# Artemarius/cuda-gaussian-splatting

Hardware: AMD Instinct MI355X
Metric: fwd+bwd Mpixels/s @1080p, 1M Gaussians, SH3 (higher is better)
Workload: dtype f32

## Files before the change

cuda-gaussian-splatting_amd/csrc/sort_bin.h:

```cpp
#pragma once

#include "sort_bin_cover.h"
#include "sort_tile_order.h"

namespace {

constexpr int BIN_WAVES = 16, BIN_NT = BIN_WAVES * CUGS_WAVE;
inline uint32_t bin_window_groups(int ntx) { const uint32_t nbx = ((uint32_t)ntx + 7u) / 8u; return (nbx + 7u) / 8u; }
inline uint32_t bin_window_cols(int ntx) {
    const uint32_t nbx = ((uint32_t)ntx + 7u) / 8u, gxs = bin_window_groups(ntx);
    return ((nbx + gxs - 1u) / gxs) * 8u;
}
inline uint32_t bin_windows(int ntx, int nty) { return (((uint32_t)nty + 7u) / 8u) * bin_window_groups(ntx); }

constexpr int BIN_D_MAX = BIN_TILES_CAP + 2 * CUGS_PRECT_MAX_TILES + 2;
__global__ __launch_bounds__(BIN_NT) void k_bin_count(uint32_t n, uint32_t group, const uint32_t* __restrict__ order,
                                                      const int4* __restrict__ rect, const uint32_t* __restrict__ prect_in,
                                                      uint32_t* __restrict__ prect_out, uint32_t ntx, uint32_t nty,
                                                      uint32_t* __restrict__ table, uint32_t* __restrict__ zero_pairs,
                                                      uint32_t* __restrict__ win) {
    __shared__ int32_t s_d[BIN_D_MAX];
    if (blockIdx.x == 0 && threadIdx.x < BIN_WINDOWS_MAX) win[threadIdx.x] = 0u;
    __shared__ int32_t s_part[8][128];
    const uint32_t tid = threadIdx.x, wave = tid >> 6, lane = tid & 63u;
    const uint32_t w2 = ntx + 1u, cells = w2 * (nty + 1u);
    for (uint32_t e = tid; e < cells; e += BIN_NT) s_d[e] = 0;
    __syncthreads();
    const uint32_t base = blockIdx.x * group;
    const uint32_t end = min(n, base + group);
    for (uint32_t i = base + tid; i < end; i += BIN_NT) {
        uint32_t pr;
        if (prect_in) {
            pr = prect_in[i];
        } else {
            pr = pack_rect(rect[order[i]]);
            prect_out[i] = pr;
        }
        if (pr & 0x80000000u) {
            const uint32_t z = pr & 0x7FFFFFFFu;
            if (z) atomicAdd(zero_pairs, z);
            continue;
        }
        const uint32_t x0 = pr & 127u, y0 = (pr >> 7) & 127u, w = (pr >> 14) & 127u, h = (pr >> 21) & 127u;
        atomicAdd(&s_d[y0 * w2 + x0], 1);
        atomicAdd(&s_d[y0 * w2 + x0 + w], -1);
        atomicAdd(&s_d[(y0 + h) * w2 + x0], -1);
        atomicAdd(&s_d[(y0 + h) * w2 + x0 + w], 1);
    }
    __syncthreads();
    for (uint32_t row = wave; row < nty; row += BIN_WAVES) {
        int32_t carry = 0;
        for (uint32_t c0 = 0; c0 < ntx; c0 += CUGS_WAVE) {
            const uint32_t x = c0 + lane;
            const int32_t v = x < ntx ? s_d[row * w2 + x] : 0;
            const int32_t inc = (int32_t)wave_inclusive_scan((uint32_t)v) + carry;
            if (x < ntx) s_d[row * w2 + x] = inc;
            carry = __shfl(inc, 63);
        }
    }
    __syncthreads();
    {
        const uint32_t x = tid & 127u, seg = tid >> 7;
        const uint32_t rps = (nty + 7u) / 8u;
        const uint32_t ya = min(nty, seg * rps), yb = min(nty, ya + rps);
        int32_t sum = 0;
        if (x < ntx)
            for (uint32_t y = ya; y < yb; ++y) sum += s_d[y * w2 + x];
        s_part[seg][x] = sum;
        __syncthreads();
        int32_t run = 0;
        for (uint32_t s2 = 0; s2 < seg; ++s2) run += s_part[s2][x];
        if (x < ntx)
            for (uint32_t y = ya; y < yb; ++y) {
                run += s_d[y * w2 + x];
                s_d[y * w2 + x] = run;
            }
    }
    __syncthreads();
    uint32_t* out = table + (size_t)blockIdx.x * (ntx * nty);
    for (uint32_t row = wave; row < nty; row += BIN_WAVES)
        for (uint32_t x = lane; x < ntx; x += CUGS_WAVE) out[row * ntx + x] = (uint32_t)s_d[row * w2 + x];
}

__global__ __launch_bounds__(BIN_NT) void k_bin_scan(uint32_t rows, uint32_t tiles, uint32_t* __restrict__ table,
                                                     uint32_t* __restrict__ ttot, uint32_t* __restrict__ tpre,
                                                     uint32_t* __restrict__ csum, uint32_t* __restrict__ q12,
                                                     uint32_t* __restrict__ range_flag, uint32_t* __restrict__ snap,
                                                     uint32_t* __restrict__ win, uint32_t ntx, uint32_t win_cols,
                                                     uint32_t gxs) {
    __shared__ uint32_t s_seg[BIN_WAVES][CUGS_WAVE];
    __shared__ uint32_t s_win[BIN_WINDOWS_MAX];
    if (blockIdx.x == 0 && threadIdx.x == 0) {
        snap[0] = q12[0]; q12[1] = q12[0]; q12[0] = 0u;
        snap[1] = *range_flag; *range_flag = 0u;
    }
    const uint32_t tl = threadIdx.x & 63u, seg = threadIdx.x >> 6;
    const uint32_t t = blockIdx.x * CUGS_WAVE + tl;
    const uint32_t rps = (rows + BIN_WAVES - 1u) / BIN_WAVES;
    const uint32_t r0 = min(rows, seg * rps), r1 = min(rows, r0 + rps);
    uint32_t sum = 0u;
    if (t < tiles) {
#pragma unroll 8
        for (uint32_t r = r0; r < r1; ++r) sum += table[(size_t)r * tiles + t];
    }
    s_seg[seg][tl] = sum;
    __syncthreads();
    uint32_t pre = 0u, tot = 0u;
#pragma unroll
    for (uint32_t s2 = 0; s2 < (uint32_t)BIN_WAVES; ++s2) {
        const uint32_t v = s_seg[s2][tl];
        pre += s2 < seg ? v : 0u;
        tot += v;
    }
    if (t < tiles) {
        uint32_t run = pre;
#pragma unroll 8
        for (uint32_t r = r0; r < r1; ++r) {
            const uint32_t v = table[(size_t)r * tiles + t];
            table[(size_t)r * tiles + t] = run;
            run += v;
        }
    }
    if (seg == 0u) {
        const uint32_t v = t < tiles ? tot : 0u;
        const uint32_t inc = wave_inclusive_scan(v);
        if (t < tiles) { ttot[t] = v; tpre[t] = inc - v; }
        if (tl == 63u) csum[blockIdx.x] = inc;
        if (win) {
            s_win[tl] = 0u;
            __builtin_amdgcn_fence(__ATOMIC_ACQ_REL, "wavefront");
            __builtin_amdgcn_wave_barrier();
            if (v) {
                const uint32_t ty = t / ntx, tx = t - ty * ntx;
                atomicAdd(&s_win[(ty >> 3) * gxs + tx / win_cols], v);
            }
            __builtin_amdgcn_fence(__ATOMIC_ACQ_REL, "wavefront");
            __builtin_amdgcn_wave_barrier();
            const uint32_t mine = s_win[tl];
            if (mine) atomicAdd(&win[tl], mine);
        }
    }
}

constexpr int BIN_BLK = 8;
constexpr int BIN_WG_WAVES = 8;
constexpr int BIN_SLICE = 512;
constexpr int BIN_SLICE_STEPS = BIN_SLICE / CUGS_WAVE;
constexpr int BIN_RUN = 16;
constexpr int BIN_RUN_STRIDE = BIN_RUN + 3;
__device__ __forceinline__ void bin_wave_lds_sync() {
    __builtin_amdgcn_fence(__ATOMIC_ACQ_REL, "wavefront");
    __builtin_amdgcn_wave_barrier();
}
template <int CTRL>
__device__ __forceinline__ uint32_t bin_dpp(uint32_t v) {
    return (uint32_t)__builtin_amdgcn_update_dpp(0, (int)v, CTRL, 0xF, 0xF, false);
}
template <int S, uint32_t M>
__device__ __forceinline__ uint32_t bin_tr_merge(uint32_t v, uint32_t p, bool upper) {
    const uint32_t keep = upper ? ~M : M;
    const uint32_t moved = __builtin_rotateright32(p, upper ? (uint32_t)S : 32u - (uint32_t)S);
    return (v & keep) | (moved & ~keep);
}
__device__ __forceinline__ void bin_transpose64(uint32_t& lo, uint32_t& hi, uint32_t lane) {
    {
        const auto r = __builtin_amdgcn_permlane32_swap(lo, hi, false, false);
        lo = r[0]; hi = r[1];
    }
    {
        const bool up = (lane & 16u) != 0u;
        const uint32_t pl = (uint32_t)__shfl_xor((int)lo, 16), ph = (uint32_t)__shfl_xor((int)hi, 16);
        lo = bin_tr_merge<16, 0x0000FFFFu>(lo, pl, up); hi = bin_tr_merge<16, 0x0000FFFFu>(hi, ph, up);
    }
    {
        const bool up = (lane & 8u) != 0u;
        const uint32_t pl = bin_dpp<0x128>(lo), ph = bin_dpp<0x128>(hi);
        lo = bin_tr_merge<8, 0x00FF00FFu>(lo, pl, up); hi = bin_tr_merge<8, 0x00FF00FFu>(hi, ph, up);
    }
    {
        const bool up = (lane & 4u) != 0u;
        const uint32_t pl = bin_dpp<0x1B>(bin_dpp<0x141>(lo)), ph = bin_dpp<0x1B>(bin_dpp<0x141>(hi));
        lo = bin_tr_merge<4, 0x0F0F0F0Fu>(lo, pl, up); hi = bin_tr_merge<4, 0x0F0F0F0Fu>(hi, ph, up);
    }
    {
        const bool up = (lane & 2u) != 0u;
        const uint32_t pl = bin_dpp<0x4E>(lo), ph = bin_dpp<0x4E>(hi);
        lo = bin_tr_merge<2, 0x33333333u>(lo, pl, up); hi = bin_tr_merge<2, 0x33333333u>(hi, ph, up);
    }
    {
        const bool up = (lane & 1u) != 0u;
        const uint32_t pl = bin_dpp<0xB1>(lo), ph = bin_dpp<0xB1>(hi);
        lo = bin_tr_merge<1, 0x55555555u>(lo, pl, up); hi = bin_tr_merge<1, 0x55555555u>(hi, ph, up);
    }
}
__device__ __forceinline__ void bin_pop_batch(const uint2* hits, uint32_t count, uint32_t lane, uint32_t blk_tx0,
                                              uint32_t blk_ty0, bool tile_ok, char* outb, uint32_t& pos) {
    bin_wave_lds_sync();
    const uint64_t cover = lane < count ? bin_cover_mask(hits[lane].x, blk_tx0, blk_ty0) : 0ull;
    uint32_t lo = (uint32_t)cover, hi = (uint32_t)(cover >> 32);
    bin_transpose64(lo, hi, lane);
    if (!tile_ok) lo = hi = 0u;
    const uint32_t* const word = reinterpret_cast<const uint32_t*>(hits);
    while (lo != 0u) {
        const uint32_t b = (uint32_t)__builtin_ctz(lo);
        lo &= lo - 1u;
        *reinterpret_cast<uint32_t*>(outb + pos) = word[2u * b + 1u];
        pos += 4u;
    }
    while (hi != 0u) {
        const uint32_t b = (uint32_t)__builtin_ctz(hi);
        hi &= hi - 1u;
        *reinterpret_cast<uint32_t*>(outb + pos) = word[2u * b + 65u];
        pos += 4u;
    }
    bin_wave_lds_sync();
}

template <bool STAGE>
__global__ __launch_bounds__(BIN_WG_WAVES * CUGS_WAVE) void k_bin_scatter(
    uint32_t n, uint32_t group, uint32_t nbx, uint32_t nby, uint32_t gxs, uint32_t pairs_or_cap, bool predicted,
    const uint32_t* __restrict__ order, const uint32_t* __restrict__ prect, uint32_t ntx, uint32_t nty,
    const uint32_t* __restrict__ table, const uint32_t* __restrict__ ttot, const uint32_t* __restrict__ tpre,
    const uint32_t* __restrict__ csum, const uint32_t* __restrict__ snap, uint32_t* __restrict__ tbase,
    unsigned long long* __restrict__ total, unsigned long long* __restrict__ total_mapped, uint32_t* __restrict__ out,
    int32_t* __restrict__ tile_ranges, uint32_t* __restrict__ tile_order, const uint32_t* __restrict__ win) {
    __shared__ uint2 s_cand[BIN_WG_WAVES][BIN_SLICE];
    __shared__ uint32_t s_cnt[BIN_WG_WAVES];
    __shared__ uint2 s_hit[STAGE ? 1 : BIN_WG_WAVES * CUGS_WAVE];
    __shared__ uint32_t s_run[STAGE ? BIN_WG_WAVES * CUGS_WAVE * BIN_RUN_STRIDE + 4 : 1];
    const uint32_t nt = blockDim.x, nw = nt >> 6, tid = threadIdx.x, wid = tid >> 6, lane = tid & 63u;
    const uint32_t per_group = nby * gxs;
    uint32_t blk = blockIdx.x / per_group, rem = blockIdx.x - blk * per_group;
    const uint32_t win_mine = (win && lane < per_group) ? win[lane] : 0u;
    const uint32_t zero = snap[0];
    const bool bad = snap[1] != 0u;
    const uint32_t tiles = ntx * nty;

    const uint32_t nch = (tiles + CUGS_WAVE - 1u) / CUGS_WAVE;
    uint32_t cpre[3] = {0u, 0u, 0u};
    uint32_t pairs = zero;
#pragma unroll
    for (int i = 0; i < 3; ++i) {
        if ((uint32_t)i * CUGS_WAVE < nch) {
            const uint32_t c = lane + (uint32_t)i * CUGS_WAVE;
            const uint32_t v = c < nch ? csum[c] : 0u;
            uint32_t inc = v;
#pragma unroll
            for (int d = 1; d < 64; d <<= 1) {
                const uint32_t o = __shfl_up(inc, d);
                const uint32_t sum = inc + o;
                if ((int)lane >= d) inc = sum < o ? 0xFFFFFFFFu : sum;
            }
            const uint32_t with = inc + pairs;
            cpre[i] = (with < inc ? 0xFFFFFFFFu : with) - v;
            const uint32_t last = __shfl(inc, 63), tot = last + pairs;
            pairs = tot < last ? 0xFFFFFFFFu : tot;
        }
    }
    const bool fits = !bad && (!predicted || pairs <= pairs_or_cap);
    cpre[0] -= zero; cpre[1] -= zero; cpre[2] -= zero;
    if (__ballot((unsigned long long)win_mine * per_group > 2ull * pairs) != 0ull) {
        uint32_t rank = 0u;
        for (uint32_t w2 = 0; w2 < per_group; ++w2) {
            const uint32_t o = (uint32_t)__builtin_amdgcn_readlane((int)win_mine, (int)w2);
            rank += (o > win_mine || (o == win_mine && w2 < lane)) ? 1u : 0u;
        }
        const uint32_t groups = gridDim.x / per_group;
        const uint32_t slot = blockIdx.x / groups;
        blk = blockIdx.x - slot * groups;
        rem = (uint32_t)__builtin_ctzll(__ballot(lane < per_group && rank == slot));
    }
    const uint32_t by = rem / gxs, gx = rem - by * gxs;

    const uint32_t bx = gx * nw + wid;
    const bool active = bx < nbx;
    const uint32_t tx = bx * BIN_BLK + (lane & 7u), ty = by * BIN_BLK + (lane >> 3);
    const bool tile_ok = active && tx < ntx && ty < nty;
    const uint32_t t = tile_ok ? ty * ntx + tx : 0u;
    uint32_t start;
    {
        const uint32_t ch = t >> 6;
        const uint32_t p0 = __shfl(cpre[0], ch & 63u), p1 = __shfl(cpre[1], ch & 63u), p2 = __shfl(cpre[2], ch & 63u);
        start = zero + (ch < 64u ? p0 : ch < 128u ? p1 : p2) + (tile_ok ? tpre[t] : 0u);
    }
    uint32_t pos = tile_ok ? (start + table[(size_t)blk * tiles + t]) * 4u : 0u;
    if (blk == 0u) {
        if (tile_ok) {
            const uint32_t c = fits ? ttot[t] + (t == 0u ? zero : 0u) : 0u;
            tile_ranges[2 * t + 0] = c ? (int32_t)(t == 0u ? 0u : start) : 0;
            tile_ranges[2 * t + 1] = c ? (int32_t)(start + ttot[t]) : 0;
            tbase[t] = start;
        }
        if (rem == 0u && tid == 0u) {
            unsigned long long exact = zero;
            for (uint32_t c = 0; c < nch; ++c) exact += csum[c];
            tbase[tiles] = pairs;
            const unsigned long long host_total = bad ? ~0ull : exact;
            total[0] = bad ? 0ull : exact;
            total[1] = host_total;
            if (total_mapped) __hip_atomic_store(total_mapped, host_total, __ATOMIC_RELAXED, __HIP_MEMORY_SCOPE_SYSTEM);
        }
    }
    if (tile_order && blockIdx.x == 0u) {
        uint32_t* const s_lds = reinterpret_cast<uint32_t*>(&s_cand[0][0]);
        uint32_t* const s_chunk = s_lds + ORDER_LDS;
        if (wid == 0u) {
#pragma unroll
            for (int i = 0; i < 3; ++i)
                if (lane + (uint32_t)i * CUGS_WAVE < nch) s_chunk[lane + (uint32_t)i * CUGS_WAVE] = cpre[i];
        }
        write_tile_order(tiles, [&](uint32_t t2) { return fits ? ttot[t2] + (t2 == 0u ? zero : 0u) : 0u; },
                         [&](uint32_t t2) { return t2 == 0u ? 0u : zero + s_chunk[t2 >> 6] + tpre[t2]; },
                         reinterpret_cast<uint4*>(tile_order), s_lds);
    }
    if (!fits) return;
    if (blk == 0u)
        for (uint32_t k = rem * nt + tid; k < zero; k += per_group * nt) out[k] = 0u;
    const uint32_t win_y0 = by * BIN_BLK, win_y1 = win_y0 + BIN_BLK;
    const uint32_t win_x0 = gx * nw * BIN_BLK, win_x1 = win_x0 + nw * BIN_BLK;
    const uint32_t blk_x0 = bx * BIN_BLK, blk_x1 = blk_x0 + BIN_BLK;
    const unsigned long long lt_mask = (1ull << lane) - 1ull;
    char* const outb = reinterpret_cast<char*>(out);
    uint32_t* const run = s_run + (STAGE ? tid * BIN_RUN_STRIDE : 0u);
    uint32_t held = 0u;
    uint2* const hits = s_hit + (STAGE ? 0u : wid * CUGS_WAVE);
    uint32_t nhit = 0u;
    const uint32_t base = blk * group;
    const uint32_t end = min(n, base + group);
    const uint32_t stage = nw * BIN_SLICE;
    for (uint32_t c0 = base; c0 < end; c0 += stage) {
        __syncthreads();
        {
            const uint32_t s_begin = c0 + wid * BIN_SLICE;
            uint32_t pr[BIN_SLICE_STEPS], gq[BIN_SLICE_STEPS];
            bool ov[BIN_SLICE_STEPS];
#pragma unroll
            for (int u = 0; u < BIN_SLICE_STEPS; ++u) {
                const uint32_t i = s_begin + (uint32_t)u * CUGS_WAVE + lane;
                pr[u] = prect[min(i, end - 1u)];
                gq[u] = order[min(i, end - 1u)];
                if (i >= end) pr[u] = 0x80000000u;
            }
#pragma unroll
            for (int u = 0; u < BIN_SLICE_STEPS; ++u) {
                const uint32_t x0 = pr[u] & 127u, y0 = (pr[u] >> 7) & 127u, w = (pr[u] >> 14) & 127u, h = (pr[u] >> 21) & 127u;
                ov[u] = (int32_t)pr[u] >= 0 && y0 < win_y1 && y0 + h > win_y0 && x0 < win_x1 && x0 + w > win_x0;
            }
            uint32_t found = 0u;
#pragma unroll
            for (int u = 0; u < BIN_SLICE_STEPS; ++u) {
                const unsigned long long m = __ballot(ov[u]);
                if (ov[u]) s_cand[wid][found + (uint32_t)__popcll(m & lt_mask)] = make_uint2(pr[u], gq[u]);
                found += (uint32_t)__popcll(m);
            }
            if (lane == 0u) s_cnt[wid] = found;
        }
        __syncthreads();
        if (!active) continue;
        if constexpr (!STAGE) {
            const uint32_t cnts = s_cnt[lane & (uint32_t)(BIN_WG_WAVES - 1)];
            for (uint32_t w2 = 0; w2 < nw; ++w2) {
                const uint32_t c = (uint32_t)__builtin_amdgcn_readlane((int)cnts, (int)w2);
                for (uint32_t k0 = 0; k0 < c; k0 += CUGS_WAVE) {
                    const uint2 rec = s_cand[w2][k0 + lane];
                    const uint32_t x0v = rec.x & 127u, wv = (rec.x >> 14) & 127u;
                    const bool hit = k0 + lane < c && (int32_t)rec.x >= 0 && x0v < blk_x1 && x0v + wv > blk_x0;
                    const unsigned long long m = __builtin_amdgcn_ballot_w64(hit);
                    const uint32_t slot = __builtin_amdgcn_mbcnt_hi((uint32_t)(m >> 32), __builtin_amdgcn_mbcnt_lo((uint32_t)m, nhit));
                    if (hit && slot < (uint32_t)CUGS_WAVE) hits[slot] = rec;
                    nhit = (uint32_t)__builtin_amdgcn_readfirstlane((int)(nhit + (uint32_t)__popcll(m)));
                    if (nhit >= (uint32_t)CUGS_WAVE) {
                        bin_pop_batch(hits, (uint32_t)CUGS_WAVE, lane, blk_x0, win_y0, tile_ok, outb, pos);
                        if (hit && slot >= (uint32_t)CUGS_WAVE) hits[slot - (uint32_t)CUGS_WAVE] = rec;
                        nhit -= (uint32_t)CUGS_WAVE;
                    }
                }
            }
            continue;
        }
        for (uint32_t w2 = 0; w2 < nw; ++w2) {
            const uint32_t c = s_cnt[w2];
            for (uint32_t k0 = 0; k0 < c; k0 += CUGS_WAVE) {
                uint2 rec = make_uint2(0x80000000u, 0u);
                if (k0 + lane < c) rec = s_cand[w2][k0 + lane];
                const uint32_t x0v = rec.x & 127u, wv = (rec.x >> 14) & 127u;
                unsigned long long m = __ballot((int32_t)rec.x >= 0 && x0v < blk_x1 && x0v + wv > blk_x0);
                while (m != 0ull) {
                    const int l = __builtin_ctzll(m);
                    m &= m - 1ull;
                    const uint32_t prl = (uint32_t)__builtin_amdgcn_readlane((int)rec.x, l);
                    const uint32_t g = (uint32_t)__builtin_amdgcn_readlane((int)rec.y, l);
                    const uint32_t x0 = prl & 127u, y0 = (prl >> 7) & 127u, w = (prl >> 14) & 127u, h = (prl >> 21) & 127u;
                    const bool in = ((tx - x0) < w) & ((ty - y0) < h);
                    if constexpr (STAGE) {
                        if (in) run[held++] = g;
                        if (__ballot(held == (uint32_t)BIN_RUN) != 0ull) {
                            const uint32_t whole = held & ~3u;
#pragma unroll
                            for (int q = 0; q < BIN_RUN; q += 4)
                                if ((uint32_t)q < whole)
                                    *reinterpret_cast<uint4*>(outb + pos + 4 * q) = make_uint4(run[q], run[q + 1], run[q + 2], run[q + 3]);
                            const uint32_t rest = held - whole;
                            const uint32_t r0 = run[whole], r1 = run[whole + 1u], r2 = run[whole + 2u];
                            if (rest > 0u) run[0] = r0;
                            if (rest > 1u) run[1] = r1;
                            if (rest > 2u) run[2] = r2;
                            pos += 4u * whole;
                            held = rest;
                        }
                    } else if (in) {
                        *reinterpret_cast<uint32_t*>(outb + pos) = g;
                        pos += 4u;
                    }
                }
            }
        }
    }
    if constexpr (!STAGE) {
        if (nhit != 0u) bin_pop_batch(hits, nhit, lane, blk_x0, win_y0, tile_ok, outb, pos);
    }
    if constexpr (STAGE) {
        for (uint32_t q = 0; __ballot(q < held) != 0ull; ++q)
            if (q < held) *reinterpret_cast<uint32_t*>(outb + pos + 4u * q) = run[q];
    }
}

__global__ __launch_bounds__(CUGS_BLOCK) void k_bin_keys(uint32_t pairs_or_cap, const unsigned long long* __restrict__ dev_count,
                                                         uint32_t tiles, const uint32_t* __restrict__ tbase,
                                                         const uint32_t* __restrict__ zero_snap,
                                                         const int32_t* __restrict__ pidx, const float* __restrict__ depths,
                                                         uint64_t* __restrict__ keys_sorted) {
    if (dev_count && *dev_count > (unsigned long long)pairs_or_cap) return;
    const uint32_t total = live_count(pairs_or_cap, dev_count);
    const uint32_t i = blockIdx.x * CUGS_BLOCK + threadIdx.x;
    if (i >= total) return;
    if (i < *zero_snap) { keys_sorted[i] = 0ull; return; }
    uint32_t lo = 0u, hi = tiles;
    while (hi - lo > 1u) {
        const uint32_t mid = (lo + hi) >> 1;
        if (tbase[mid] <= i) lo = mid; else hi = mid;
    }
    keys_sorted[i] = ((uint64_t)lo << 32) | (uint64_t)__float_as_uint(depths[pidx[i]]);
}

}
```

cuda-gaussian-splatting_amd/csrc/sort_radix.h:

```cpp
#pragma once

#include "sort_workspace.h"

namespace {

__device__ __forceinline__ uint32_t wave_inclusive_scan(uint32_t v) {
    const int lane = threadIdx.x & 63;
#pragma unroll
    for (int d = 1; d < 64; d <<= 1) {
        uint32_t t = __shfl_up(v, d);
        if (lane >= d) v += t;
    }
    return v;
}

template <int NW = 4>
__device__ __forceinline__ uint32_t block_exclusive_scan(uint32_t v, uint32_t* s_tmp, uint32_t* total) {
    const int lane = threadIdx.x & 63, wave = threadIdx.x >> 6;
    uint32_t inc = wave_inclusive_scan(v);
    if (lane == 63) s_tmp[wave] = inc;
    __syncthreads();
    uint32_t base = 0, sum = 0;
#pragma unroll
    for (int w = 0; w < NW; ++w) {
        const uint32_t t = s_tmp[w];
        base += (w < wave) ? t : 0u;
        sum += t;
    }
    if (total) *total = sum;
    __syncthreads();
    return base + inc - v;
}

__device__ __forceinline__ uint32_t live_count(uint32_t count, const unsigned long long* __restrict__ dev_count) {
    if (!dev_count) return count;
    const unsigned long long t = *dev_count;
    return t < (unsigned long long)count ? (uint32_t)t : count;
}

template <typename K, int NT, int CHUNK, int RDX = RADIX>
__global__ __launch_bounds__(NT) void k_radix_hist(const K* __restrict__ keys, uint32_t count_or_cap,
                                                   const unsigned long long* __restrict__ dev_count, int shift,
                                                   uint32_t mask, uint32_t* __restrict__ hist, uint32_t nblk,
                                                   uint32_t* __restrict__ ctl, uint32_t* __restrict__ sup, uint32_t sb) {
    const uint32_t count = live_count(count_or_cap, dev_count);
    constexpr int PER = CHUNK / NT;
    constexpr int NWORDS = PER * (int)sizeof(K) / 4;
    static_assert(NWORDS >= 2 && NWORDS * 4 == PER * (int)sizeof(K), "whole 8-byte loads per thread");
    static_assert(NT >= RDX, "one thread per digit");
    __shared__ uint32_t s_cnt[RDX];
    if (threadIdx.x < RDX) s_cnt[threadIdx.x] = 0;
    if (ctl && blockIdx.x == 0 && threadIdx.x == 0) { ctl[1] = ctl[0]; ctl[0] = 0u; }
    __syncthreads();
    const uint32_t bbase = blockIdx.x * CHUNK;
    if (bbase + CHUNK <= count) {
        uint32_t wds[NWORDS];
        if constexpr (NWORDS % 4 == 0) {
            const uint4* src = reinterpret_cast<const uint4*>(keys + bbase + threadIdx.x * PER);
#pragma unroll
            for (int v = 0; v < NWORDS / 4; ++v) {
                const uint4 q = src[v];
                wds[4 * v] = q.x; wds[4 * v + 1] = q.y; wds[4 * v + 2] = q.z; wds[4 * v + 3] = q.w;
            }
        } else {
            const uint2* src = reinterpret_cast<const uint2*>(keys + bbase + threadIdx.x * PER);
#pragma unroll
            for (int v = 0; v < NWORDS / 2; ++v) {
                const uint2 q = src[v];
                wds[2 * v] = q.x; wds[2 * v + 1] = q.y;
            }
        }
#pragma unroll
        for (int c = 0; c < NWORDS; ++c) {
            if (sizeof(K) == 4) {
                atomicAdd(&s_cnt[(wds[c] >> shift) & mask], 1u);
            } else {
                atomicAdd(&s_cnt[((wds[c] & 0xFFFFu) >> shift) & mask], 1u);
                atomicAdd(&s_cnt[((wds[c] >> 16) >> shift) & mask], 1u);
            }
        }
    } else {
        for (uint32_t i = bbase + threadIdx.x; i < count; i += NT)
            atomicAdd(&s_cnt[((uint32_t)keys[i] >> shift) & mask], 1u);
    }
    __syncthreads();
    if (threadIdx.x < RDX) {
        const uint32_t c = s_cnt[threadIdx.x];
        if (sup) {
            hist[(size_t)blockIdx.x * RDX + threadIdx.x] = c;
            if (c) atomicAdd(&sup[(size_t)(blockIdx.x / sb) * RDX + threadIdx.x], c);
        } else {
            hist[(size_t)threadIdx.x * nblk + blockIdx.x] = c;
        }
    }
}

__global__ __launch_bounds__(CUGS_BLOCK) void k_radix_scan_rows(const uint32_t* hist, uint32_t* out,
                                                                uint32_t nblk, uint32_t* __restrict__ tot) {
    __shared__ uint32_t s_tmp[4];
    constexpr int PER = 8;
    const uint32_t* row = hist + (size_t)blockIdx.x * nblk;
    uint32_t* orow = out + (size_t)blockIdx.x * nblk;
    uint32_t carry = 0;
    for (uint32_t base = 0; base < nblk; base += CUGS_BLOCK * PER) {
        const uint32_t i0 = base + threadIdx.x * PER;
        uint32_t v[PER], sum = 0;
#pragma unroll
        for (int e = 0; e < PER; ++e) { v[e] = (i0 + e < nblk) ? row[i0 + e] : 0u; sum += v[e]; }
        uint32_t total;
        uint32_t run = carry + block_exclusive_scan(sum, s_tmp, &total);
#pragma unroll
        for (int e = 0; e < PER; ++e) {
            if (i0 + e < nblk) orow[i0 + e] = run;
            run += v[e];
        }
        carry += total;
    }
    if (threadIdx.x == 0) tot[blockIdx.x] = carry;
}

template <typename K, bool IOTA, int NB, int NT, bool ARANK, int CHUNK, int RDX = RADIX, bool V2 = false>
__global__ __launch_bounds__(NT) void k_radix_scatter(
    const K* __restrict__ keys_in, const uint32_t* __restrict__ vals_in, uint32_t count_or_cap,
    const unsigned long long* __restrict__ dev_count, int shift, uint32_t mask_rt, const uint32_t* __restrict__ hist,
    const uint32_t* __restrict__ sup, uint32_t sb, const uint32_t* __restrict__ tot, uint32_t nblk,
    K* __restrict__ keys_out, uint32_t* __restrict__ vals_out,
    const uint32_t* __restrict__ vals2_in = nullptr, uint32_t* __restrict__ vals2_out = nullptr) {
    const uint32_t mask = ARANK ? mask_rt : ((1u << NB) - 1u);
    const uint32_t count = live_count(count_or_cap, dev_count);
    if (blockIdx.x * CHUNK >= count) return;
    constexpr int NW = NT / CUGS_WAVE;
    constexpr int PER = CHUNK / NT;
    constexpr int SLICE = CUGS_WAVE * PER;
    static_assert(NT >= RDX && (1 << NB) <= RDX, "one thread per digit");
    __shared__ uint32_t s_lbase[NW][RDX];
    __shared__ uint32_t s_lstart[RDX];
    __shared__ uint32_t s_gbase[RDX];
    __shared__ K s_key[CHUNK];
    __shared__ uint32_t s_val[CHUNK];
    __shared__ uint32_t s_val2[V2 ? CHUNK : 1];
    __shared__ uint32_t s_tmp[NW];
    const uint32_t tid = threadIdx.x, wave = tid >> 6, lane = tid & 63;
    const uint32_t bbase = blockIdx.x * CHUNK;
    const uint32_t wbase = bbase + wave * SLICE;
    const uint32_t count_blk = min((uint32_t)CHUNK, count - bbase);

    constexpr int ND = ARANK ? RDX : (1 << NB);
    constexpr int GRP = NT / ND;
    uint32_t pre = 0u, totd = 0u;
    if (sup) {
        const uint32_t d = tid % ND, part = tid / ND;
        const uint32_t mysb = blockIdx.x / sb, nsb = (nblk + sb - 1u) / sb;
#pragma unroll 4
        for (uint32_t r = part; r < nsb; r += GRP) {
            const uint32_t v = sup[(size_t)r * RDX + d];
            totd += v;
            pre += (r < mysb) ? v : 0u;
        }
#pragma unroll 4
        for (uint32_t b2 = mysb * sb + part; b2 < blockIdx.x; b2 += GRP) pre += hist[(size_t)b2 * RDX + d];
    } else if (tid < RDX) {
        pre = hist[(size_t)tid * nblk + blockIdx.x];
        totd = tot[tid];
    }

    for (uint32_t e = tid; e < NW * RDX; e += NT) (&s_lbase[0][0])[e] = 0;
    if (tid < RDX) { s_gbase[tid] = 0u; s_lstart[tid] = 0u; }
    __syncthreads();
    if (sup && GRP > 1) {
        if (pre) atomicAdd(&s_gbase[tid % ND], pre);
        if (totd) atomicAdd(&s_lstart[tid % ND], totd);
    } else if (tid < RDX) {
        s_gbase[tid] = pre; s_lstart[tid] = totd;
    }

    uint32_t k[PER], v[PER], v2[V2 ? PER : 1];
#pragma unroll
    for (int r = 0; r < PER; ++r) {
        uint32_t i = wbase + r * CUGS_WAVE + lane;
        bool ok = i < count;
        k[r] = ok ? (uint32_t)__builtin_nontemporal_load(keys_in + i) : 0xFFFFFFFFu;
        v[r] = ok ? (IOTA ? i : __builtin_nontemporal_load(vals_in + i)) : 0u;
        if constexpr (V2) v2[r] = ok ? __builtin_nontemporal_load(vals2_in + i) : 0u;
        if (ok) atomicAdd(&s_lbase[wave][(k[r] >> shift) & mask], 1u);
    }
    __syncthreads();

    {
        const bool dig = tid < RDX;
        uint32_t cnt = 0;
        if (dig) {
#pragma unroll
            for (int w = 0; w < NW; ++w) cnt += s_lbase[w][tid];
        }
        const uint32_t before = dig ? s_gbase[tid] : 0u;
        const uint32_t dig_base = block_exclusive_scan<NW>(dig ? s_lstart[tid] : 0u, s_tmp, nullptr);
        const uint32_t lstart = block_exclusive_scan<NW>(cnt, s_tmp, nullptr);
        if (dig) {
            s_gbase[tid] = dig_base + before;
            s_lstart[tid] = lstart;
            uint32_t run = lstart;
#pragma unroll
            for (int w = 0; w < NW; ++w) {
                const uint32_t c = s_lbase[w][tid];
                s_lbase[w][tid] = run;
                run += c;
            }
        }
    }
    __syncthreads();

    const unsigned long long lt_mask = (1ull << lane) - 1ull;
#pragma unroll
    for (int r = 0; r < PER; ++r) {
        const uint32_t i = wbase + r * CUGS_WAVE + lane;
        const bool ok = i < count;
        const uint32_t d = (k[r] >> shift) & mask;
        if constexpr (ARANK) {
            if (ok) {
                const uint32_t pos = atomicAdd(&s_lbase[wave][d], 1u);
                s_key[pos] = (K)k[r];
                s_val[pos] = v[r];
                if constexpr (V2) s_val2[pos] = v2[r];
            }
            continue;
        }
        unsigned long long peers = __ballot(ok);
#pragma unroll
        for (int b = 0; b < NB; ++b) {
            const bool bit = (d >> b) & 1u;
            const unsigned long long m = __ballot(bit);
            peers &= bit ? m : ~m;
        }
        if (ok) {
            const uint32_t base = s_lbase[wave][d];
            const uint32_t pos = base + __popcll(peers & lt_mask);
            s_key[pos] = (K)k[r];
            s_val[pos] = v[r];
            if constexpr (V2) s_val2[pos] = v2[r];
            if ((peers >> lane) == 1ull) s_lbase[wave][d] = base + __popcll(peers);
        }
    }
    __syncthreads();

#pragma unroll
    for (int r = 0; r < PER; ++r) {
        const uint32_t j = r * NT + tid;
        if (j < count_blk) {
            const K key = s_key[j];
            const uint32_t d = ((uint32_t)key >> shift) & mask;
            const uint32_t dst = s_gbase[d] + (j - s_lstart[d]);
            keys_out[dst] = key;
            vals_out[dst] = s_val[j];
            if constexpr (V2) vals2_out[dst] = s_val2[j];
        }
    }
}

#ifdef CUGS_DEV
__device__ __forceinline__ uint32_t probe_digit(uint32_t set, uint32_t wave, uint32_t r, uint32_t lane) {
    uint32_t h = (set * 4u + wave) * 8u + r;
    h = (h ^ 61u) ^ (h >> 16); h *= 9u; h ^= h >> 4; h *= 0x27d4eb2du; h ^= h >> 15;
    uint32_t x = h + lane * 0x9E3779B9u;
    x ^= x >> 16; x *= 0x7feb352du; x ^= x >> 15; x *= 0x846ca68bu; x ^= x >> 16;
    switch (set % 6u) {
        case 0: return x & 255u;
        case 1: return x & 127u;
        case 2: return x & 3u;
        case 3: return 5u;
        case 4: return (x & 1u) ? 7u : 39u;
        default: return (lane * 37u + (x & 1u)) & 63u;
    }
}
__global__ __launch_bounds__(CUGS_BLOCK) void k_probe_lds_order(uint32_t* __restrict__ violations) {
    __shared__ uint32_t cnt[4][RADIX];
    const uint32_t wave = threadIdx.x >> 6, lane = threadIdx.x & 63, set = blockIdx.x;
    for (uint32_t i = threadIdx.x; i < 4 * RADIX; i += CUGS_BLOCK) (&cnt[0][0])[i] = 0;
    __syncthreads();
    uint32_t d[8], got[8];
#pragma unroll
    for (int r = 0; r < 8; ++r) d[r] = probe_digit(set, wave, r, lane);
#pragma unroll
    for (int r = 0; r < 8; ++r) got[r] = atomicAdd(&cnt[wave][d[r]], 1u);
    uint32_t bad = 0;
    for (int r = 0; r < 8; ++r) {
        uint32_t expect = 0;
        for (int rr = 0; rr <= r; ++rr)
            for (uint32_t l = 0; l < 64u && !(rr == r && l >= lane); ++l) expect += probe_digit(set, wave, rr, l) == d[r];
        bad += expect != got[r];
    }
    if (bad) atomicAdd(violations, bad);
}
#endif

template <typename K, bool IOTA, int NT, int CHUNK, int RDX = RADIX>
int radix_pass(const K* kin, const uint32_t* vin, uint32_t count, const unsigned long long* dev_count, int shift, int bits,
               uint32_t* hist, uint32_t* sup, uint32_t* tot, K* kout, uint32_t* vout, uint32_t* ctl, hipStream_t st,
               const uint32_t* v2in = nullptr, uint32_t* v2out = nullptr) {
    const uint32_t nblk = nblocks_for(count, CHUNK);
    const uint32_t sb = sup_block(nblk);
    static_assert(NT % RDX == 0, "whole thread groups per digit");
    if (!scan_free(nblk, (uint32_t)NT >> bits)) sup = nullptr;
    hipLaunchKernelGGL((k_radix_hist<K, NT, CHUNK, RDX>), dim3(nblk), dim3(NT), 0, st, kin, count, dev_count, shift,
                       (1u << bits) - 1u, hist, nblk, ctl, sup, sb);
    CUGS_LAUNCH_CHECK();
    if (!sup) {
        hipLaunchKernelGGL(k_radix_scan_rows, dim3(RDX), dim3(CUGS_BLOCK), 0, st, hist, hist, nblk, tot);
        CUGS_LAUNCH_CHECK();
    }
    if constexpr (RDX == RADIX_DEPTH) {
        if (v2in)
            hipLaunchKernelGGL((k_radix_scatter<K, IOTA, DEPTH_BITS, NT, false, CHUNK, RDX, true>), dim3(nblk), dim3(NT), 0, st, kin,
                               vin, count, dev_count, shift, 0u, hist, sup, sb, tot, nblk, kout, vout, v2in, v2out);
        else
            hipLaunchKernelGGL((k_radix_scatter<K, IOTA, DEPTH_BITS, NT, false, CHUNK, RDX>), dim3(nblk), dim3(NT), 0, st, kin, vin, count,
                               dev_count, shift, 0u, hist, sup, sb, tot, nblk, kout, vout);
        CUGS_LAUNCH_CHECK();
        return 0;
    }
    if (v2in) return CUGS_EINVAL;
#ifdef CUGS_DEV
    if (rank_mode() == 1) {
        hipLaunchKernelGGL((k_radix_scatter<K, IOTA, 8, NT, true, CHUNK>), dim3(nblk), dim3(NT), 0, st, kin, vin, count, dev_count,
                           shift, (1u << bits) - 1u, hist, sup, sb, tot, nblk, kout, vout);
        CUGS_LAUNCH_CHECK();
        return 0;
    }
#endif
#define CUGS_SCATTER(NB)                                                                                          \
    hipLaunchKernelGGL((k_radix_scatter<K, IOTA, NB, NT, false, CHUNK>), dim3(nblk), dim3(NT), 0, st, kin, vin, count, dev_count, \
                       shift, 0u, hist, sup, sb, tot, nblk, kout, vout)
    switch (bits) {
        case 1: CUGS_SCATTER(1); break;
        case 2: CUGS_SCATTER(2); break;
        case 3: CUGS_SCATTER(3); break;
        case 4: CUGS_SCATTER(4); break;
        case 5: CUGS_SCATTER(5); break;
        case 6: CUGS_SCATTER(6); break;
        case 7: CUGS_SCATTER(7); break;
        default: CUGS_SCATTER(8); break;
    }
#undef CUGS_SCATTER
    CUGS_LAUNCH_CHECK();
    return 0;
}

}
```

Before: 2730.

## Hoist global loads ahead of shared-memory init in bin count, bin scan, and radix scatter

In k_bin_count the per-thread rect/prect loads are issued into registers before the shared histogram is zeroed and the barrier is taken, so load latency overlaps the init. k_bin_scan now loads a fixed number of rows per thread into registers once via templated unrolling, so the second pass does not re-read global memory. The radix scatter kernel issues key/value loads before the shared-memory clear and fuses two block scans into one pass with a single barrier. The cost is more register pressure, which may lower occupancy, plus clamped out-of-range loads.

```diff
diff --git a/cuda-gaussian-splatting_amd/csrc/sort_bin.h b/cuda-gaussian-splatting_amd/csrc/sort_bin.h
--- a/cuda-gaussian-splatting_amd/csrc/sort_bin.h
+++ b/cuda-gaussian-splatting_amd/csrc/sort_bin.h
@@ -6,6 +6,8 @@
 namespace {
 
 constexpr int BIN_WAVES = 16, BIN_NT = BIN_WAVES * CUGS_WAVE;
+constexpr uint32_t BIN_SCAN_ROWS = BIN_ROWS_MAX / BIN_WAVES;
+static_assert(BIN_ROWS_MAX % BIN_WAVES == 0 && BIN_GROUP % BIN_NT == 0, "whole rows per wave, whole records per thread");
 inline uint32_t bin_window_groups(int ntx) { const uint32_t nbx = ((uint32_t)ntx + 7u) / 8u; return (nbx + 7u) / 8u; }
 inline uint32_t bin_window_cols(int ntx) {
     const uint32_t nbx = ((uint32_t)ntx + 7u) / 8u, gxs = bin_window_groups(ntx);
@@ -14,6 +16,19 @@
 inline uint32_t bin_windows(int ntx, int nty) { return (((uint32_t)nty + 7u) / 8u) * bin_window_groups(ntx); }
 
 constexpr int BIN_D_MAX = BIN_TILES_CAP + 2 * CUGS_PRECT_MAX_TILES + 2;
+constexpr int BIN_PER = (int)BIN_GROUP / BIN_NT;
+__device__ __forceinline__ void bin_count_add(uint32_t pr, int32_t* s_d, uint32_t w2, uint32_t* __restrict__ zero_pairs) {
+    if (pr & 0x80000000u) {
+        const uint32_t z = pr & 0x7FFFFFFFu;
+        if (z) atomicAdd(zero_pairs, z);
+        return;
+    }
+    const uint32_t x0 = pr & 127u, y0 = (pr >> 7) & 127u, w = (pr >> 14) & 127u, h = (pr >> 21) & 127u;
+    atomicAdd(&s_d[y0 * w2 + x0], 1);
+    atomicAdd(&s_d[y0 * w2 + x0 + w], -1);
+    atomicAdd(&s_d[(y0 + h) * w2 + x0], -1);
+    atomicAdd(&s_d[(y0 + h) * w2 + x0 + w], 1);
+}
 __global__ __launch_bounds__(BIN_NT) void k_bin_count(uint32_t n, uint32_t group, const uint32_t* __restrict__ order,
                                                       const int4* __restrict__ rect, const uint32_t* __restrict__ prect_in,
                                                       uint32_t* __restrict__ prect_out, uint32_t ntx, uint32_t nty,
@@ -24,28 +39,46 @@
     __shared__ int32_t s_part[8][128];
     const uint32_t tid = threadIdx.x, wave = tid >> 6, lane = tid & 63u;
     const uint32_t w2 = ntx + 1u, cells = w2 * (nty + 1u);
+    const uint32_t base = blockIdx.x * group;
+    const uint32_t end = min(n, base + group);
+    const bool whole = group == BIN_GROUP;
+    uint32_t pr[BIN_PER];
+    if (whole) {
+        if (prect_in) {
+#pragma unroll
+            for (int u = 0; u < BIN_PER; ++u) pr[u] = prect_in[min(base + (uint32_t)u * BIN_NT + tid, end - 1u)];
+        } else {
+            uint32_t g[BIN_PER];
+#pragma unroll
+            for (int u = 0; u < BIN_PER; ++u) g[u] = order[min(base + (uint32_t)u * BIN_NT + tid, end - 1u)];
+            int4 rc[BIN_PER];
+#pragma unroll
+            for (int u = 0; u < BIN_PER; ++u) rc[u] = rect[g[u]];
+#pragma unroll
+            for (int u = 0; u < BIN_PER; ++u) {
+                const uint32_t i = base + (uint32_t)u * BIN_NT + tid;
+                pr[u] = pack_rect(rc[u]);
+                if (i < end) prect_out[i] = pr[u];
+            }
+        }
+    }
     for (uint32_t e = tid; e < cells; e += BIN_NT) s_d[e] = 0;
     __syncthreads();
-    const uint32_t base = blockIdx.x * group;
-    const uint32_t end = min(n, base + group);
-    for (uint32_t i = base + tid; i < end; i += BIN_NT) {
-        uint32_t pr;
-        if (prect_in) {
-            pr = prect_in[i];
-        } else {
-            pr = pack_rect(rect[order[i]]);
-            prect_out[i] = pr;
-        }
-        if (pr & 0x80000000u) {
-            const uint32_t z = pr & 0x7FFFFFFFu;
-            if (z) atomicAdd(zero_pairs, z);
-            continue;
-        }
-        const uint32_t x0 = pr & 127u, y0 = (pr >> 7) & 127u, w = (pr >> 14) & 127u, h = (pr >> 21) & 127u;
-        atomicAdd(&s_d[y0 * w2 + x0], 1);
-        atomicAdd(&s_d[y0 * w2 + x0 + w], -1);
-        atomicAdd(&s_d[(y0 + h) * w2 + x0], -1);
-        atomicAdd(&s_d[(y0 + h) * w2 + x0 + w], 1);
+    if (whole) {
+#pragma unroll
+        for (int u = 0; u < BIN_PER; ++u)
+            if (base + (uint32_t)u * BIN_NT + tid < end) bin_count_add(pr[u], s_d, w2, zero_pairs);
+    } else {
+        for (uint32_t i = base + tid; i < end; i += BIN_NT) {
+            uint32_t p;
+            if (prect_in) {
+                p = prect_in[i];
+            } else {
+                p = pack_rect(rect[order[i]]);
+                prect_out[i] = p;
+            }
+            bin_count_add(p, s_d, w2, zero_pairs);
+        }
     }
     __syncthreads();
     for (uint32_t row = wave; row < nty; row += BIN_WAVES) {
@@ -82,6 +115,47 @@
         for (uint32_t x = lane; x < ntx; x += CUGS_WAVE) out[row * ntx + x] = (uint32_t)s_d[row * w2 + x];
 }
 
+template <int R>
+__device__ __forceinline__ uint32_t bin_scan_run(uint32_t* __restrict__ table, uint32_t rows, uint32_t tiles, uint32_t t,
+                                                 uint32_t r0, uint32_t r1, uint32_t (*s_seg)[CUGS_WAVE], uint32_t seg,
+                                                 uint32_t tl) {
+    uint32_t col[R];
+    const uint32_t tc = min(t, tiles - 1u), rlast = rows ? rows - 1u : 0u;
+#pragma unroll
+    for (int j = 0; j < R; ++j) col[j] = table[min(r0 + (uint32_t)j, rlast) * tiles + tc];
+    uint32_t sum = 0u;
+#pragma unroll
+    for (int j = 0; j < R; ++j) {
+        if (r0 + (uint32_t)j >= r1 || t >= tiles) col[j] = 0u;
+        sum += col[j];
+    }
+    for (uint32_t r = r0 + (uint32_t)R; r < r1; ++r)
+        if (t < tiles) sum += table[r * tiles + t];
+    s_seg[seg][tl] = sum;
+    __syncthreads();
+    uint32_t pre = 0u, tot = 0u;
+#pragma unroll
+    for (uint32_t s2 = 0; s2 < (uint32_t)BIN_WAVES; ++s2) {
+        const uint32_t v = s_seg[s2][tl];
+        pre += s2 < seg ? v : 0u;
+        tot += v;
+    }
+    if (t < tiles) {
+        uint32_t run = pre;
+#pragma unroll
+        for (int j = 0; j < R; ++j) {
+            if (r0 + (uint32_t)j < r1) table[(r0 + (uint32_t)j) * tiles + t] = run;
+            run += col[j];
+        }
+        for (uint32_t r = r0 + (uint32_t)R; r < r1; ++r) {
+            const uint32_t v = table[r * tiles + t];
+            table[r * tiles + t] = run;
+            run += v;
+        }
+    }
+    return tot;
+}
+
 __global__ __launch_bounds__(BIN_NT) void k_bin_scan(uint32_t rows, uint32_t tiles, uint32_t* __restrict__ table,
                                                      uint32_t* __restrict__ ttot, uint32_t* __restrict__ tpre,
                                                      uint32_t* __restrict__ csum, uint32_t* __restrict__ q12,
@@ -98,29 +172,10 @@
     const uint32_t t = blockIdx.x * CUGS_WAVE + tl;
     const uint32_t rps = (rows + BIN_WAVES - 1u) / BIN_WAVES;
     const uint32_t r0 = min(rows, seg * rps), r1 = min(rows, r0 + rps);
-    uint32_t sum = 0u;
-    if (t < tiles) {
-#pragma unroll 8
-        for (uint32_t r = r0; r < r1; ++r) sum += table[(size_t)r * tiles + t];
-    }
-    s_seg[seg][tl] = sum;
-    __syncthreads();
-    uint32_t pre = 0u, tot = 0u;
-#pragma unroll
-    for (uint32_t s2 = 0; s2 < (uint32_t)BIN_WAVES; ++s2) {
-        const uint32_t v = s_seg[s2][tl];
-        pre += s2 < seg ? v : 0u;
-        tot += v;
-    }
-    if (t < tiles) {
-        uint32_t run = pre;
-#pragma unroll 8
-        for (uint32_t r = r0; r < r1; ++r) {
-            const uint32_t v = table[(size_t)r * tiles + t];
-            table[(size_t)r * tiles + t] = run;
-            run += v;
-        }
-    }
+    const uint32_t tot = rps <= 4u ? bin_scan_run<4>(table, rows, tiles, t, r0, r1, s_seg, seg, tl)
+                       : rps <= 8u ? bin_scan_run<8>(table, rows, tiles, t, r0, r1, s_seg, seg, tl)
+                       : rps <= 16u ? bin_scan_run<16>(table, rows, tiles, t, r0, r1, s_seg, seg, tl)
+                       : bin_scan_run<(int)BIN_SCAN_ROWS>(table, rows, tiles, t, r0, r1, s_seg, seg, tl);
     if (seg == 0u) {
         const uint32_t v = t < tiles ? tot : 0u;
         const uint32_t inc = wave_inclusive_scan(v);
diff --git a/cuda-gaussian-splatting_amd/csrc/sort_radix.h b/cuda-gaussian-splatting_amd/csrc/sort_radix.h
--- a/cuda-gaussian-splatting_amd/csrc/sort_radix.h
+++ b/cuda-gaussian-splatting_amd/csrc/sort_radix.h
@@ -30,6 +30,27 @@
     if (total) *total = sum;
     __syncthreads();
     return base + inc - v;
+}
+
+template <int NW>
+__device__ __forceinline__ void block_exclusive_scan2(uint32_t& a, uint32_t& b, uint32_t* s_tmp) {
+    const int lane = threadIdx.x & 63, wave = threadIdx.x >> 6;
+    uint32_t ia = a, ib = b;
+#pragma unroll
+    for (int d = 1; d < 64; d <<= 1) {
+        const uint32_t ta = __shfl_up(ia, d), tb = __shfl_up(ib, d);
+        if (lane >= d) { ia += ta; ib += tb; }
+    }
+    if (lane == 63) { s_tmp[wave] = ia; s_tmp[NW + wave] = ib; }
+    __syncthreads();
+    uint32_t base_a = 0, base_b = 0;
+#pragma unroll
+    for (int w = 0; w < NW; ++w) {
+        base_a += (w < wave) ? s_tmp[w] : 0u;
+        base_b += (w < wave) ? s_tmp[NW + w] : 0u;
+    }
+    a = base_a + ia - a;
+    b = base_b + ib - b;
 }
 
 __device__ __forceinline__ uint32_t live_count(uint32_t count, const unsigned long long* __restrict__ dev_count) {
@@ -139,7 +160,7 @@
     __shared__ K s_key[CHUNK];
     __shared__ uint32_t s_val[CHUNK];
     __shared__ uint32_t s_val2[V2 ? CHUNK : 1];
-    __shared__ uint32_t s_tmp[NW];
+    __shared__ uint32_t s_tmp[2 * NW];
     const uint32_t tid = threadIdx.x, wave = tid >> 6, lane = tid & 63;
     const uint32_t bbase = blockIdx.x * CHUNK;
     const uint32_t wbase = bbase + wave * SLICE;
@@ -163,27 +184,34 @@
         pre = hist[(size_t)tid * nblk + blockIdx.x];
         totd = tot[tid];
     }
+    uint32_t k[PER], v[PER], v2[V2 ? PER : 1];
+#pragma unroll
+    for (int r = 0; r < PER; ++r) {
+        const uint32_t i = min(wbase + r * CUGS_WAVE + lane, count - 1u);
+        k[r] = (uint32_t)__builtin_nontemporal_load(keys_in + i);
+        if constexpr (!IOTA) v[r] = __builtin_nontemporal_load(vals_in + i);
+        if constexpr (V2) v2[r] = __builtin_nontemporal_load(vals2_in + i);
+    }
 
     for (uint32_t e = tid; e < NW * RDX; e += NT) (&s_lbase[0][0])[e] = 0;
     if (tid < RDX) { s_gbase[tid] = 0u; s_lstart[tid] = 0u; }
     __syncthreads();
+
+#pragma unroll
+    for (int r = 0; r < PER; ++r) {
+        const uint32_t i = wbase + r * CUGS_WAVE + lane;
+        const bool ok = i < count;
+        if (!ok) k[r] = 0xFFFFFFFFu;
+        if constexpr (IOTA) v[r] = ok ? i : 0u; else if (!ok) v[r] = 0u;
+        if constexpr (V2) { if (!ok) v2[r] = 0u; }
+        if (ok) atomicAdd(&s_lbase[wave][(k[r] >> shift) & mask], 1u);
+    }
     if (sup && GRP > 1) {
         if (pre) atomicAdd(&s_gbase[tid % ND], pre);
         if (totd) atomicAdd(&s_lstart[tid % ND], totd);
     } else if (tid < RDX) {
         s_gbase[tid] = pre; s_lstart[tid] = totd;
     }
-
-    uint32_t k[PER], v[PER], v2[V2 ? PER : 1];
-#pragma unroll
-    for (int r = 0; r < PER; ++r) {
-        uint32_t i = wbase + r * CUGS_WAVE + lane;
-        bool ok = i < count;
-        k[r] = ok ? (uint32_t)__builtin_nontemporal_load(keys_in + i) : 0xFFFFFFFFu;
-        v[r] = ok ? (IOTA ? i : __builtin_nontemporal_load(vals_in + i)) : 0u;
-        if constexpr (V2) v2[r] = ok ? __builtin_nontemporal_load(vals2_in + i) : 0u;
-        if (ok) atomicAdd(&s_lbase[wave][(k[r] >> shift) & mask], 1u);
-    }
     __syncthreads();
 
     {
@@ -194,8 +222,8 @@
             for (int w = 0; w < NW; ++w) cnt += s_lbase[w][tid];
         }
         const uint32_t before = dig ? s_gbase[tid] : 0u;
-        const uint32_t dig_base = block_exclusive_scan<NW>(dig ? s_lstart[tid] : 0u, s_tmp, nullptr);
-        const uint32_t lstart = block_exclusive_scan<NW>(cnt, s_tmp, nullptr);
+        uint32_t dig_base = dig ? s_lstart[tid] : 0u, lstart = cnt;
+        block_exclusive_scan2<NW>(dig_base, lstart, s_tmp);
         if (dig) {
             s_gbase[tid] = dig_base + before;
             s_lstart[tid] = lstart;
```

Result: no change. 2737, median of 2 (+0.2%).
